# Ignalina/znippy

Hardware: AMD Instinct MI355X
Metric: decompress MB/s (uncompressed) + compress MB/s, 100k x 10KB archive (higher is better)
Workload: dtype u8; 1 GPU; 100k x 10KiB text chunks (BASELINE configs[1]); rows_per_gpu=100000, chunk_bytes=10240, bytes_per_gpu=1024000000, blob_bytes_per_gpu=6400000, parallelism=row-cursor ranges x1, pipelining=step k+1 queued before step k's counters are read (two runs in flight)

## Files before the change

znippy_amd/csrc/api.hip:

```cpp
#include <unistd.h>
#include "common.h"
#include "encode.h"
#include "../../include/znippy_hip.h"

#include <algorithm>
#include <cstdio>
#include <cstdlib>
#include <cstring>
#include <chrono>
#include <memory>
#include <string>
#include <vector>
#include <unordered_map>

namespace zn {
int measure_b3_pass_ns(int cus, hipStream_t s, float *ns_per_pass_per_simd, float *ghz);
size_t decode_lit_scratch_bytes(int grid);
void set_fused_dbg(unsigned long long *p);
void set_fused_abl(int v);
}

using namespace zn;
extern "C" void zn_rounds_totals(const uint64_t *len, const uint8_t *skip, size_t n, uint64_t out[8]);
extern "C" void zn_rows_extents(const uint64_t *bo, const uint64_t *bs, const uint64_t *oo, const uint64_t *us, size_t n, uint64_t out[8]);
// ... 59 lines not shown
    uint16_t *bx_fse_pool = nullptr;
    uint16_t *bx_huf_pool = nullptr;
    uint64_t bx_fse_cap = 0, bx_huf_cap = 0;
    uint32_t *rx_pool = nullptr, *rx_chunk = nullptr;
    uint8_t *rx_cdone = nullptr;
    uint64_t rx_cap = 0;
    uint8_t *vs_pool = nullptr;
    uint64_t vs_cap = 0;
    hipEvent_t ev_fork = nullptr, ev_join = nullptr, ev_join2 = nullptr;
    std::vector<KTime> ktimes;
    int n_ktimes = 0;
    std::vector<hipEvent_t> event_pool;
    bool ktime_open = false;
    std::vector<std::pair<size_t, void *>> pinned_pool;
    size_t pinned_pool_bytes = 0;
    std::vector<std::pair<size_t, void *>> dev_pool;
    std::unordered_map<void *, size_t> dev_sizes;
    size_t dev_pool_bytes = 0;
    struct {
        int dbg = 0;
        unsigned lds_pad = 0;
        int store_g = 0;
        bool no_block_items = false, no_fused_blocks = false, ddbg = false, edbg = false, no_fused_store = false,
             nohash = false, no_roles = false, no_fz = false, fz_only = false, no_bx = false, tdbg = false, no_fuse_hash = false, trace = false, no_rx = false, no_pack = false, no_lean = false, no_stored_only = false;
        unsigned roles_min = 2048;
        unsigned bx_big = BX_BIG_SEQ;
        bool bx_big_set = false;
        int ktime = 2;
    } sw;
    int cus = 256;
    int live_tables = 0;
    bool closing = false;
    unsigned long long *clk_buf = nullptr;
    enum Diag { DIAG_FUSED, DIAG_ITEMS, DIAG_FZ, DIAG_GENERAL, DIAG_BX, DIAG_ENCODE, DIAG_N };
    unsigned long long *diag[DIAG_N] = {};
};

static void read_switches(znippy_ctx *ctx) {
    auto on = [](const char *n) { const char *v = getenv(n); return v && *v && *v != '0'; };
    if (const char *e = getenv("ZNIPPY_DBG")) ctx->sw.dbg = atoi(e);
    if (const char *e = getenv("ZNIPPY_LDS_PAD")) ctx->sw.lds_pad = (unsigned)atoi(e);
    ctx->sw.no_block_items = on("ZNIPPY_NO_BLOCK_ITEMS");
    ctx->sw.no_fused_blocks = on("ZNIPPY_NO_FUSED_BLOCKS");
    ctx->sw.ddbg = on("ZNIPPY_DDBG");
    ctx->sw.edbg = on("ZNIPPY_EDBG");
    ctx->sw.no_fused_store = on("ZNIPPY_NO_FUSED_STORE");
    ctx->sw.nohash = on("ZNIPPY_NOHASH");
    ctx->sw.no_roles = on("ZNIPPY_NO_ROLES");
    ctx->sw.no_fz = on("ZNIPPY_NO_FZ");
    ctx->sw.tdbg = on("ZNIPPY_TDBG");
    ctx->sw.trace = on("ZNIPPY_TRACE");
    ctx->sw.no_lean = on("ZNIPPY_NO_LEAN");
    ctx->sw.no_pack = on("ZNIPPY_NO_PACK");
    if (const char *e = getenv("ZNIPPY_STORE_G")) ctx->sw.store_g = atoi(e) == 1 ? 1 : (atoi(e) == 2 ? 2 : 0);
    ctx->sw.no_stored_only = on("ZNIPPY_NO_STORED_ONLY");
    ctx->sw.no_rx = on("ZNIPPY_NO_RX");
    ctx->sw.no_fuse_hash = on("ZNIPPY_NO_FUSE_HASH");
    ctx->sw.no_bx = on("ZNIPPY_NO_BX");
    if (const char *e = getenv("ZNIPPY_BX_BIG")) { ctx->sw.bx_big = (unsigned)atoi(e); ctx->sw.bx_big_set = true; }
    if (const char *lv = getenv("ZNIPPY_LEVEL")) { const int v = atoi(lv); if (v >= 1 && v <= 22) ctx->level = v; }
    if (const char *wl = getenv("ZNIPPY_WINDOW_LOG")) { const int v = atoi(wl); if (v == 0 || (v >= WINDOW_LOG_MIN && v <= WINDOW_LOG_MAX)) ctx->window_log = v; }
    if (const char *gs = getenv("ZNIPPY_GEN_SHARE")) { const int v = atoi(gs); if (v >= 1 && v <= 4) ctx->gen_share = v; }
    ctx->sw.fz_only = on("ZNIPPY_FZ_ONLY");
    if (const char *e = getenv("ZNIPPY_ROLES_MIN")) ctx->sw.roles_min = (unsigned)atoi(e);
    if (const char *e = getenv("ZNIPPY_KTIME")) ctx->sw.ktime = atoi(e);
}

static void *pinned_take(znippy_ctx *ctx, size_t bytes, size_t *cap) {
    size_t best = ctx->pinned_pool.size();
    for (size_t i = 0; i < ctx->pinned_pool.size(); i++)
        if (ctx->pinned_pool[i].first >= bytes && ctx->pinned_pool[i].first <= 4 * bytes + 4096 &&
            (best == ctx->pinned_pool.size() || ctx->pinned_pool[i].first < ctx->pinned_pool[best].first))
            best = i;
    if (best != ctx->pinned_pool.size()) {
        void *p = ctx->pinned_pool[best].second;
// ... 180 lines not shown
    H_ITEMS = 2,
    H_TILES = 3,
    H_FLAGGED = 5,
};
enum Cursor : uint32_t { CUR_GENERAL = 0, CUR_ROLES = 2, CUR_ITEMS = 4, CUR_FALLBACK = 8, CUR_FZ = 12, CUR_FZ_WORK = 13 };
constexpr uint32_t LEAN_ANY = 1u << H_FUSED | 1u << H_SERIAL | 1u << H_FLAGGED, LEAN_SMALL = LEAN_ANY | 1u << H_TILES, LEAN_BLOCKS = LEAN_ANY | 1u << H_ITEMS;
constexpr bool ctl_before(CtlRegion a, CtlRegion b) { return a.at + a.bytes <= b.at; }
static_assert(ctl_before(CTL_COUNTERS, CTL_HAND) && ctl_before(CTL_HAND, CTL_CURSORS) && ctl_before(CTL_CURSORS, CTL_FZ_POOL) && ctl_before(CTL_FZ_POOL, CTL_BX_POOL) &&
              ctl_before(CTL_BX_POOL, CTL_BX_CTR) && ctl_before(CTL_BX_CTR, CTL_RX) && CTL_RX.at + CTL_RX.bytes <= CTL_HEAD, "control block: regions overlap or pass the head");
static_assert(CTL_COUNTERS.at == 0 && CTL_HAND.at == CTL_COUNTERS.bytes && CTL_MIRROR == CTL_HAND.at + CTL_HAND.bytes, "the mirror is exactly counters + hand-over counts");
static_assert(CTL_FLAG < 8 && H_FLAGGED == H_SERIAL + 4 && H_FLAGGED < 8 && CUR_FZ_WORK < 16 && zn::RX_ROUNDS <= RX_ZERO && RX_ZERO < 16, "control block: a word outside its region");

struct znippy_rows {
    znippy_ctx *ctx = nullptr;
    uint64_t row_begin = 0;
    uint32_t n = 0;
    uint32_t n_compressed = 0;
    uint64_t *blob_off = nullptr, *blob_size = nullptr, *usize = nullptr, *out_off = nullptr;
    uint8_t *compressed = nullptr, *checksum = nullptr, *d_bitmap = nullptr;
    uint32_t *h_pack = nullptr, *d_pack = nullptr;
    size_t h_pack_cap = 0;
    unsigned long long *d_pack_sums = nullptr;
    uint8_t *ctl = nullptr;
    size_t ctl_bytes = 0;
    template <class T> T *ctl_at(CtlRegion g, size_t i = 0) const { return reinterpret_cast<T *>(ctl + g.at) + i; }
    uint32_t *hand(Hand h) const { return ctl_at<uint32_t>(CTL_HAND, h); }
    uint32_t *cur(Cursor c) const { return ctl_at<uint32_t>(CTL_CURSORS, c); }
    int32_t *status = nullptr;
    uint32_t *digests = nullptr;
    uint64_t *counters = nullptr;
    uint64_t *h_counters = nullptr;
    const uint32_t *mirror_hand(unsigned slot) const { return reinterpret_cast<const uint32_t *>(reinterpret_cast<const uint8_t *>(h_counters + 16 * slot) + CTL_HAND.at); }
    size_t h_counters_cap = 0;
    int bx_hint = -1;
    bool lean_ok = false;
    int lean_hint = -1;
    bool lean_blocks_ok = false;
    bool lean_mixed_ok = false;
    bool roles_off = false;
    bool small_ok = false, small_off = false;
    uint32_t *all_rows = nullptr;
    int lean_hint2 = -1;
    struct RunArgs { const void *blobs = nullptr; void *out = nullptr; uint64_t base = 0, cap = 0, blob_cap = ~0ull; bool verify = false; } run_args[2];
    uint64_t *vs_off = nullptr;
    uint64_t vs_bytes = 0;
    bool vs_built = false;
    bool no_out = false;
    hipEvent_t ev_done[2] = {nullptr, nullptr};
    uint64_t run_seq = 0;
    uint64_t ext_min_bo = 0, ext_max_bend = 0, ext_max_oend = 0;
    bool ext_wrap = false;
    std::vector<uint64_t> h_blob_off, h_blob_size, h_len, h_out_off;
    uint64_t blob_cap = ~0ull;
    uint64_t val_base = 0, val_bcap = 0, val_ocap = 0;
    bool val_done = false, val_verify = false;
    uint32_t n_bad = 0;
    bool force_full = false;
    uint8_t *status_init = nullptr;
// ... 805 lines not shown
    r->ctx = ctx;
    ctx->live_tables++;
    r->row_begin = row_begin;
    r->n = (uint32_t)(row_end - row_begin);
    const uint32_t n = r->n;
    bool allc = true;
    if (compressed_bitmap) {
        uint64_t row = row_begin;
        for (; row < row_end && (row & 7); row++) allc &= (compressed_bitmap[row >> 3] >> (row & 7)) & 1;
        for (; row + 8 <= row_end && allc; row += 8) allc &= compressed_bitmap[row >> 3] == 0xFF;
        for (; row < row_end && allc; row++) allc &= (compressed_bitmap[row >> 3] >> (row & 7)) & 1;
    }
    std::vector<uint64_t> own_oo;
    if (!out_offset) {
        r->no_out = true;
        own_oo.resize(n);
        uint64_t at = 0;
        for (uint32_t i = 0; i < n; i++) { own_oo[i] = at; at += uncompressed_size[row_begin + i]; }
    }
    const RowCols c{blob_offset + row_begin, blob_size + row_begin, uncompressed_size + row_begin, out_offset ? out_offset + row_begin : own_oo.data(), compressed_bitmap, row_begin, row_end, allc};
    int rc = rows_columns_h2d(ctx, r, c, checksum, td);
    if (rc) return rc;
    r->corrupt_cap = std::max<uint32_t>(n, 1);
    r->ctl_bytes = CTL_HEAD + std::max<size_t>(4 * (size_t)n, 16);
    if (tmalloc(ctx, &r->ctl, r->ctl_bytes) != hipSuccess ||
        tmalloc(ctx, &r->digests, std::max<size_t>(32 * (size_t)n, 32)) != hipSuccess ||
        !(r->h_counters = (uint64_t *)pinned_take(ctx, 256, &r->h_counters_cap)) ||
        !(r->ev_done[0] = event_take(ctx)) || !(r->ev_done[1] = event_take(ctx)) ||
        tmalloc(ctx, &r->corrupt, 8 * (size_t)r->corrupt_cap) != hipSuccess)
        return ZNIPPY_E_NOMEM;
    r->counters = r->ctl_at<uint64_t>(CTL_COUNTERS);
    r->status = reinterpret_cast<int32_t *>(r->ctl + CTL_HEAD);
    td.mark("allocs");
    PlanBuf p;
    build_plan([=, us = c.us, bs = c.bs, &c](uint32_t i) -> uint64_t { return (allc || c.comp(i)) ? us[i] : bs[i]; }, n, p);
    td.mark("plan");
    if ((rc = upload_plan(ctx, p, r->plan))) return rc;
    td.mark("plan_h2d");
    for (const Tile &t : p.tiles) r->n_small_tiles += t.n_units != 0;
    if (r->n_small_tiles && tmalloc(ctx, &r->slow_list, 4 * (size_t)p.tiles.size()) != hipSuccess) return ZNIPPY_E_NOMEM;
    RowClasses k;
    rows_classify(ctx, r, c, k);
    r->n_list_a = (uint32_t)k.la.size();
    td.mark("big_rows");
    if (r->n_compressed && (rc = rows_batch_buffers(ctx, r, k.nblk))) return rc;
    r->wide_rows = k.n_big && k.big_bytes / k.n_big >= (1u << 20) && k.big_blob * 50 < k.big_bytes;
    r->n_cand = (uint32_t)k.cand_row.size();
    r->n_items = (uint32_t)k.item_row.size();
    const bool hints = !ctx->sw.no_lean && r->n_list_a == 0;
    const uint32_t n_tiles = (uint32_t)p.tiles.size();
    r->small_ok = allc && hints && !ctx->sw.no_bx && r->n_cand == 0 && r->n_small_tiles == n_tiles && r->n_small_tiles > 0 && r->bx_slots;
    r->lean_mixed_ok = hints && r->n_cand == 0 && r->n_small_tiles > 0 && r->n_small_tiles < n_tiles;
    r->lean_blocks_ok = allc && hints && r->n_cand > 0 && r->n_small_tiles == 0;
    r->lean_ok = allc && hints && r->n_cand == 0 && p.big.empty() && r->n_small_tiles == n_tiles && r->n_small_tiles > 0;
    if (r->n_cand && (rc = rows_item_buffers(ctx, r, k))) return rc;
    if (r->n_cand && !ctx->sw.no_fused_blocks && (rc = rows_fused_block_buffers(ctx, r, k, p))) return rc;
    if ((rc = dev_upload(ctx, &r->list_a, k.la.data(), k.la.size()))) return rc;
    if (tmalloc(ctx, &r->pending, std::max<size_t>(4 * (size_t)n, 16)) != hipSuccess) return ZNIPPY_E_NOMEM;
    td.mark("rest");
    *out = guard.release();
    return ZNIPPY_OK;
}
// ... 69 lines not shown
        HIPCHK(ctx, hipMemsetAsync(r->vs_off, 0, 8 * (size_t)r->n, ctx->stream));
    }
    r->vs_built = true;
    return ZNIPPY_OK;
}

static void rows_note_hint(znippy_rows *r, unsigned slot) {
    const uint32_t *left = r->mirror_hand(slot);
    const bool handed = left[H_FUSED] || left[H_SERIAL] || left[H_FLAGGED];
    r->bx_hint = (handed || r->n_list_a) ? 1 : 0;
    r->lean_hint = (handed || left[H_TILES]) ? 0 : 1;
    r->lean_hint2 = (handed || left[H_ITEMS]) ? 0 : 1;
    if (r->n_small_tiles && left[H_TILES] >= r->n_small_tiles) r->roles_off = true;
    if (r->small_ok && left[H_FUSED] >= r->n) r->small_off = true;
    if (r->small_off) r->bx_hint = 1;
}

struct RunPlan {
    bool bx;
    bool small_off;
    bool stored_only;
    bool roles;
    bool lean;
    bool lean_mixed;
    bool decode;
    bool one_stream;
    bool lean_blocks;
    bool behind;
    bool rx;
    bool third;
};
static RunPlan rows_plan(const znippy_ctx *ctx, const znippy_rows *r, int preset) {
    const auto &sw = ctx->sw;
    RunPlan p{};
    p.bx = r->bx_slots && ctx->fz_lit_pool && ctx->fz_seq_pool && ctx->bx_fse_pool && ctx->bx_huf_pool && r->bx_hint != 0;
    p.small_off = p.bx && r->small_off && !r->n_bad && !r->force_full && !sw.dbg;
    p.stored_only = r->n_compressed == 0 && !preset && !sw.dbg && !sw.no_stored_only && !r->force_full;
    const bool may_skip = !preset && !r->force_full;
    if (!p.small_off && !p.stored_only) {
        p.roles = !sw.no_roles && sw.roles_min != 0 && r->n_small_tiles >= sw.roles_min && r->n_small_tiles > 0 && !(sw.dbg & (1 | 2 | 4 | 8 | 128)) && !r->roles_off;
        p.lean_mixed = r->lean_mixed_ok && r->lean_hint == 1 && r->bx_hint == 0 && may_skip && !sw.dbg && !sw.ddbg;
        p.lean = p.roles && r->lean_ok && r->lean_hint == 1 && r->bx_hint == 0 && may_skip && !sw.dbg;
    }
    p.decode = !p.lean && !p.lean_mixed && !p.stored_only;
    if (!p.decode) return p;
    p.one_stream = r->n_cand && r->bx_hint == 0 && r->n_small_tiles == 0;
    p.lean_blocks = p.one_stream && r->lean_blocks_ok && r->lean_hint2 == 1 && may_skip && r->n_bt && !sw.ddbg && !r->fz_total;
    if (!r->n_compressed) return p;
    p.behind = !p.bx && r->n_cand && r->bx_hint == 0;
    p.rx = p.bx && r->rx_base && ctx->rx_pool && r->rx_words;
    p.third = p.bx && r->bx_nblk <= 32768;
    return p;
}

static HashArgs rows_hash_args(const znippy_ctx *ctx, const znippy_rows *r, const RowsRun &run) {
    HashArgs h{};
    h.tiles = r->plan.tiles; h.n_tiles = r->plan.n_tiles;
    h.len = r->usize;
    h.srcA = (const uint8_t *)run.d_blobs; h.offA = r->blob_off; h.baseA = run.blob_base;
    h.srcB = (uint8_t *)run.d_out; h.offB = run.verify ? r->vs_off : r->out_off;
    h.sel = r->compressed; h.status = r->status; h.pending_count = r->hand(H_FUSED);
    h.copy_to_B = run.verify ? 0 : 1;
    h.store_tiles = ctx->sw.store_g;
    h.misaligned_dst = !run.verify && (r->odd_out || ((uintptr_t)run.d_out & 15) != 0);
    h.digests = r->digests; h.tile_cv = r->plan.tile_cv;
// ... 45 lines not shown
    f.h = rows_hash_args(ctx, r, run);
    f.h.pass = 1;
    f.blob_size = r->blob_size; f.out_cap = run.out_cap; f.status = r->status;
    f.preset = run.preset;
    f.pending = r->pending; f.pending_count = r->hand(H_FUSED);
    f.dbg = ctx->sw.dbg;
    if (f.dbg & 8) {
        f.dbg_buf = diag_cycle<8>(ctx, znippy_ctx::DIAG_FUSED, s, nullptr, [](const unsigned long long *h4) {
            if (h4[3]) fprintf(stderr, "[znippy dbg] waves=%llu prologue=%.0f decode=%.0f hash=%.0f | parse+lits=%.0f expand-build=%.0f stream-out=%.0f after-match=%.0f cycles/wave\n", h4[3],
                               (double)h4[0] / h4[3], (double)h4[1] / h4[3], (double)h4[2] / h4[3], (double)h4[6] / h4[3], (double)h4[4] / h4[3], (double)h4[5] / h4[3], (double)h4[7] / h4[3]);
        });
        set_fused_dbg(f.dbg_buf);
    }
    if (f.dbg & 32768) {
        if (!ctx->clk_buf) { (void)hipMalloc(&ctx->clk_buf, 64); (void)hipMemset(ctx->clk_buf, 0, 64); }
        f.dbg_buf = ctx->clk_buf;
    }
    if (f.dbg & (16 | 32 | 64)) set_fused_abl(f.dbg);
    f.lds_pad = ctx->sw.lds_pad;
    const hipStream_t fs = p.lean_mixed ? ctx->aux : s;
    if (p.lean_mixed) {
        HIPCHK(ctx, hipEventRecord(ctx->ev_fork, s));
        HIPCHK(ctx, hipStreamWaitEvent(ctx->aux, ctx->ev_fork, 0));
    }
    if (p.roles) {
        f.cursor = r->cur(CUR_ROLES);
        f.tile_list = r->slow_list;
        f.tile_count = r->hand(H_TILES);
        timed(ctx, run.verify ? "verify_roles" : "decode_verify_roles", fs, [&] { launch_fused_roles(f, ctx->cus, fs, run.verify); });
    }
    if (r->n_small_tiles && !p.lean) timed(ctx, run.verify ? "verify_small" : "decode_verify_fused", fs, [&] { launch_fused_small(f, fs, p.roles ? ctx->cus * 5 : 0, run.verify); });
    if (p.lean_mixed) HIPCHK(ctx, hipEventRecord(ctx->ev_join, ctx->aux));
    return ZNIPPY_OK;
}

static void run_two_phase(znippy_ctx *ctx, znippy_rows *r, const RowsRun &run, hipStream_t ba) {
    FzArgs z{};
    z.cand_row = r->cand_row; z.cand_fzbase = r->fz_base; z.cand_fzcap = r->fz_cap; z.n_cand = r->n_cand;
    z.it_cand = r->fz_it_cand; z.total_items = r->fz_total; z.cand_nb = r->fz_nb; z.items = r->fz_items;
    fill_row_args(z, r, run);
    z.row_flag = r->row_flag;
    z.lit_pool = ctx->fz_lit_pool; z.lit_cap = ctx->fz_lit_cap; z.seq_pool = ctx->fz_seq_pool; z.seq_cap = ctx->fz_seq_cap;
    z.pool_used = r->ctl_at<unsigned long long>(CTL_FZ_POOL);
    z.cursor = r->cur(CUR_FZ);
    if (ctx->sw.ddbg)
        z.dbg = diag_cycle<32>(ctx, znippy_ctx::DIAG_FZ, ctx->stream, ba, [](const unsigned long long *h) {
// ... 170 lines not shown
    if (!r->n_cand) return ZNIPPY_OK;
    if (!p.behind) {
        HIPCHK(ctx, hipStreamWaitEvent(s, ctx->ev_join, 0));
        launch_finish_blocks(rows_scan_args(r, run), s, false);
    }
    decode_rest(ctx, r, a, r->n_cand);
    return ZNIPPY_OK;
}

static void run_second_hash(znippy_ctx *ctx, znippy_rows *r, const RunPlan &p, const RowsRun &run) {
    hipStream_t s = ctx->stream;
    HashArgs h = rows_hash_args(ctx, r, run);
    h.pass = p.stored_only ? 0 : 2;
    h.tile_done = r->n_bt && !p.stored_only ? r->tile_done : nullptr;
    timed(ctx, run.verify ? "blake3_hash_only" : "blake3_second_pass", s, [&] { launch_hash_tiles(h, s); });
    if (r->plan.n_big)
        timed(ctx, "blake3_merge_big", s, [&] {
            launch_merge_big(r->plan.big, r->plan.n_big, r->plan.tile_cv, r->digests, r->plan.grp_big, r->plan.grp_k, r->plan.n_grp, r->plan.max_cvs, s);
        });
}

static int run_verify(znippy_ctx *ctx, znippy_rows *r, const RunPlan &p, const RowsRun &run) {
    hipStream_t s = ctx->stream;
    if (p.lean_mixed) HIPCHK(ctx, hipStreamWaitEvent(s, ctx->ev_join, 0));
    const bool skipped = p.lean || p.lean_blocks || p.lean_mixed;
    timed(ctx, "verify", s, [&] {
        launch_verify(r->digests, r->checksum, r->usize, r->status, r->n, r->row_begin, r->counters, r->corrupt, r->corrupt_cap, s,
                      skipped ? r->ctl_at<uint32_t>(CTL_HAND) : nullptr, (p.lean || p.lean_mixed) ? LEAN_SMALL : LEAN_BLOCKS);
    });
    HIPCHK(ctx, hipMemcpyAsync(r->h_counters + 16 * run.slot, r->counters, CTL_MIRROR, hipMemcpyDeviceToHost, s));
    HIPCHK(ctx, hipEventRecord(r->ev_done[run.slot], s));
    HIPCHK(ctx, hipGetLastError());
    return ZNIPPY_OK;
}

static int rows_launch(znippy_ctx *ctx, znippy_rows *r, const void *d_blobs, uint64_t blob_base, void *d_out, uint64_t out_cap,
                       unsigned slot, bool verify, bool *queued = nullptr) {
    ctx->n_ktimes = 0;
    int rc = ensure_decoder(ctx);
    if (!rc && verify) {
        rc = rows_verify_slots(ctx, r);
        if (!rc) rc = ensure_verify_scratch(ctx, r->vs_bytes);
        d_out = ctx->vs_pool; out_cap = r->vs_bytes;
    }
    if (!rc) rc = rows_validate(ctx, r, blob_base, out_cap, verify);
    if (!rc && r->fz_total) rc = ensure_fz_pools(ctx, r->fz_bytes, r->fz_total);
// ... 665 lines not shown
```

znippy_amd/csrc/common.h:

```cpp
#pragma once
#include <hip/hip_runtime.h>
#include <stdint.h>
#include <stddef.h>

namespace zn {

struct Tile {
    uint32_t first_unit;
    uint32_t n_units;
    uint32_t first_leaf;
    uint32_t n_leaves;
    uint32_t cv_index;
    uint32_t pad;
};

struct BigUnit {
    uint32_t unit;
    uint32_t cv_base;
    uint32_t n_cvs;
    uint32_t pad;
};

struct HashArgs {
    const Tile *tiles;
// ... 26 lines not shown
    const uint32_t *pending_count;
    const uint8_t *blobs;
    uint64_t blob_base;
    const uint64_t *blob_off, *blob_size, *usize, *out_off;
    const uint8_t *compressed;
    uint8_t *out;
    uint64_t out_cap;
    int32_t *status;
    uint32_t n_rows;
    uint32_t *cursor;
    uint8_t *lit_scratch;
    unsigned long long *dbg;
    int block_mode;
    const uint32_t *item_row, *item_k;
    const uint32_t *item_src;
    uint32_t n_items;
    uint32_t *row_flag;
    const uint8_t *item_done;
    const uint32_t *todo, *n_todo;
    uint32_t *seq_scratch;
    int preset;
};

struct FusedArgs {
    HashArgs h;
    const uint64_t *blob_size;
    uint64_t out_cap;
    int32_t *status;
    uint32_t *pending;
    uint32_t *pending_count;
    int dbg;
    unsigned long long *dbg_buf;
    uint32_t lds_pad;
    int preset;
    uint32_t *cursor;
    uint32_t *tile_list;
    uint32_t *tile_count;
};

struct FusedBlocksArgs {
    HashArgs h;
    const uint64_t *blob_size;
    const uint32_t *bt_tile, *bt_item;
    uint32_t n_bt;
    const uint32_t *item_src;
    const uint32_t *row_flag;
    uint8_t *tile_done, *item_done;
    int dbg;
};
void launch_fused_blocks(const FusedBlocksArgs &a, hipStream_t s, bool verify = false);

void launch_hash_tiles(const HashArgs &a, hipStream_t s);
void launch_fused_small(const FusedArgs &a, hipStream_t s, int grid_cap = 0, bool verify = false);
void launch_fused_roles(const FusedArgs &a, int cus, hipStream_t s, bool verify = false);
void init_fused_tables();
void launch_merge_big(const BigUnit *big, uint32_t n_big, uint32_t *tile_cv, uint32_t *digests, const uint32_t *grp_big,
                      const uint32_t *grp_k, uint32_t n_grp, uint32_t max_cvs, hipStream_t s);
void launch_verify(const uint32_t *digests, const uint8_t *checksum, const uint64_t *usize,
                   const int32_t *status, uint32_t n_rows, uint64_t row_begin, uint64_t *counters,
                   uint64_t *corrupt_rows, uint32_t corrupt_cap, hipStream_t s, const uint32_t *lean_lists = nullptr, uint32_t lean_mask = 0);
int decode_grid_size(int device);
void launch_decode(const DecodeArgs &a, int grid, bool wide, hipStream_t s);
struct BlockScanArgs {
    const uint32_t *cand_row, *cand_base, *cand_nblocks;
    uint32_t n_cand;
    const uint8_t *blobs;
    uint64_t blob_base;
    const uint64_t *blob_off, *blob_size, *usize, *out_off;
    uint64_t out_cap;
    uint32_t *item_src;
    uint32_t *row_flag;
    int32_t *status;
    uint32_t *pending, *pending_count;
    int preset;
};
void launch_scan_blocks(const BlockScanArgs &a, hipStream_t s);
void launch_compact_items(const uint8_t *item_done, uint32_t n_items, uint32_t *todo, uint32_t *n_todo, hipStream_t s);
// ... 101 lines not shown
```

znippy_amd/csrc/fused_small.hip:

```cpp
#include "common.h"
#include "hash_dev.h"

#include <algorithm>
#include <cstring>

namespace zn {

constexpr uint32_t EOFF_MAX = 960;
constexpr uint32_t EBUF = EOFF_MAX + 1024 + 64;
constexpr int F_E_CORRUPT = -5, F_E_UNSUP = -6, F_E_DST = -4;
constexpr int F_NOT_SIMPLE = 1;

struct DTab {
    uint16_t next;
    uint8_t nbits, addbits;
    uint32_t base;
};
__constant__ DTab c_dll[64], c_dml[64], c_dof[32];
__constant__ uint32_t c_llb[36] = {0, 1, 2, 3, 4, 5, 6, 7, 8, 9, 10, 11, 12, 13, 14, 15, 16, 18,
                                   20, 22, 24, 28, 32, 40, 48, 64, 128, 256, 512, 1024, 2048,
                                   4096, 8192, 16384, 32768, 65536};
__constant__ uint8_t c_lla[36] = {0, 0, 0, 0, 0, 0, 0, 0, 0, 0, 0, 0, 0, 0, 0, 0, 1, 1,
                                  1, 1, 2, 2, 3, 3, 4, 6, 7, 8, 9, 10, 11, 12, 13, 14, 15, 16};
__constant__ uint32_t c_mlb[53] = {3, 4, 5, 6, 7, 8, 9, 10, 11, 12, 13, 14, 15, 16, 17, 18, 19, 20,
// ... 967 lines not shown
                else fq.fold_and_write(s_nodes, a.h);
            }
        }
        if (base + gridDim.x * 4 < n_work) lds_barrier();
    }
    if (clk) { a.dbg_buf[0] = __builtin_amdgcn_s_memtime() - c0; a.dbg_buf[1] = __builtin_amdgcn_s_memrealtime() - r0; }
}

#ifndef ZN_R_SLOTS
#define ZN_R_SLOTS 32
#endif
#ifndef ZN_R_WAVES
#define ZN_R_WAVES 16
#endif
#ifndef ZN_R_LOADERS
#define ZN_R_LOADERS 1
#endif
#ifndef ZN_R_LOADER_EMITS
#define ZN_R_LOADER_EMITS 0
#endif
constexpr uint32_t R_SLOTS = ZN_R_SLOTS, R_GROUP = 4, R_WAVES = ZN_R_WAVES, R_LOADERS = ZN_R_LOADERS;
constexpr bool R_LOADER_EMITS = ZN_R_LOADER_EMITS != 0;
static_assert((R_SLOTS & (R_SLOTS - 1)) == 0 && R_SLOTS >= 2 * R_GROUP, "ring size: a power of two, at least two groups");
constexpr uint32_t R_SLOT_BYTES = WROWS * WSTRIDE;
constexpr uint32_t R_SLOT_NODES = R_SLOT_BYTES / 32;
static_assert(R_SLOT_BYTES % 32 == 0 && R_SLOT_BYTES >= 64 * 32, "a slot must hold 64 chaining values, node-aligned");

typedef __attribute__((address_space(3))) uint32_t lds_u32;
__device__ __forceinline__ uint32_t lds_ld(const uint32_t *p) { return __builtin_amdgcn_readfirstlane(*(const volatile lds_u32 *)p); }
__device__ __forceinline__ void lds_st(uint32_t *p, uint32_t v) { *(volatile lds_u32 *)p = v; }
__device__ __forceinline__ void lds_fence() { asm volatile("s_waitcnt lgkmcnt(0)" ::: "memory"); }

struct alignas(16) RolesShared {
    uint8_t slots[R_SLOTS][R_SLOT_BYTES];
    __attribute__((aligned(16))) uint32_t tree[R_WAVES - R_LOADERS][64 * 8];
    uint64_t oo[R_SLOTS][WROWS];
    uint32_t len[R_SLOTS][WROWS];
    uint32_t tn[R_SLOTS][WROWS], toff[R_SLOTS][WROWS];
    uint16_t dy[R_SLOTS][WROWS], dB[R_SLOTS][WROWS], doff[R_SLOTS][WROWS];
    uint32_t first[R_SLOTS], nunits[R_SLOTS], nleaves[R_SLOTS];
    uint32_t ready, take, finished;
    uint32_t next_iter;
    uint32_t cnt[R_SLOTS / R_GROUP];
    uint32_t gen[R_SLOTS / R_GROUP];
};

__device__ __forceinline__ void emit_periodic_row(uint8_t *Y, uint32_t L0, uint32_t off, float inv, uint8_t *out, uint32_t osize,
                                                  uint32_t lane) {
    const uint32_t B = L0 - off, lim = L0 + 64;
    Y[L0 + lane] = Y[B + lmod(lane, off, inv)];
    const uint32_t head = (uint32_t)((16 - ((uintptr_t)out & 15)) & 15);
    const uint32_t body16 = (osize - head) >> 4;
    const uint32_t step = smod(1024, off), rb = smod(B, off);
    if (lane < head) out[lane] = Y[lane];
    const uint32_t tail = (osize - head) & 15, p = head + 16 * body16 + lane;
    if (lane < tail) {
        uint32_t rt = lmod(p, off, inv) + off - rb;
        if (rt >= off) rt -= off;
        out[p] = p < lim ? Y[p] : Y[B + rt];
    }
    uint32_t x = head + 16 * lane;
    uint32_t r = lmod(x, off, inv) + off - rb;
    if (r >= off) r -= off;
    for (uint32_t i0 = 0; i0 < body16; i0 += 256) {
        const uint32_t i = i0 + lane;
        uint4 v0 = make_uint4(0, 0, 0, 0), v1 = v0, v2 = v0, v3 = v0;
        const uint32_t r0 = r;
// ... 16 lines not shown
}

template <bool STORE>
__device__ __forceinline__ void roles_loader(const FusedArgs &a, RolesShared &S) {
    const uint32_t lane = threadIdx.x & 63, j = lane >> 4, u = lane & 15;
    FastTabs T;
    {
        const DTab eL = c_dll[lane], eM = c_dml[lane], eO = c_dof[lane & 31];
        T.ll = eL.base | (uint32_t)eL.addbits << 24;
        T.ml = eM.base | (uint32_t)eM.addbits << 24;
        T.of = eO.addbits;
        T.lls = lane < 36 ? c_llb[lane] | (uint32_t)c_lla[lane] << 24 : 0u;
        T.mls = lane < 53 ? c_mlb[lane] | (uint32_t)c_mla[lane] << 24 : 0u;
    }
    for (;;) {
        const uint32_t iter = uni(atomicAdd(&S.next_iter, lane == 0 ? 1u : 0u));
        const uint32_t base = uni(atomicAdd(a.cursor, lane == 0 ? R_GROUP : 0u));
        const bool last = base >= a.h.n_tiles;
        const uint32_t grp = iter & (R_SLOTS / R_GROUP - 1), use = iter / (R_SLOTS / R_GROUP);
        const uint32_t ti = base + j;
        Tile t{0, 0, 0, 0, 0, 0};
        if (ti < a.h.n_tiles) t = a.h.tiles[ti];
        const bool small = t.n_units >= 1;
        const bool cand = small && t.n_units <= WROWS;
        const bool rowv = cand && u < t.n_units;
        uint32_t c_sel = 0, c_bs = 0;
        uint64_t c_len = 0, c_src = 0, c_oo = 0;
        int32_t c_st = 0;
        if (rowv) {
            const uint32_t row = t.first_unit + u;
            if (a.preset) c_st = a.status[row];
            c_sel = a.h.sel[row];
            c_len = a.h.len[row];
            c_src = a.h.offA[row] - a.h.baseA;
            if (STORE) c_oo = a.h.offB[row];
            const uint64_t bs = a.blob_size[row];
            c_bs = bs > 0xFFFFFFFFull ? 0xFFFFFFFFu : (uint32_t)bs;
        }
        const bool want = rowv && c_sel && c_st == 0 && c_len != 0 && (c_len & 1023) == 0 && c_len <= 0x10000 &&
                          (!STORE || c_oo + c_len <= a.out_cap) && c_bs >= 12 && c_bs <= WIN;
        while (lds_ld(&S.gen[grp]) != use) __builtin_amdgcn_s_sleep(4);
        asm volatile("" ::: "memory");
        const uint32_t slot = grp * R_GROUP + j;
        uint8_t *const win = S.slots[slot] + (u < WROWS ? u : 0) * WSTRIDE;
        const uint8_t *const src = a.h.srcA + c_src;
        const uint32_t nb = want ? c_bs : 0, full = nb >> 4, tail = nb & 15;
// ... 251 lines not shown
            FoldQueue<4> fq;
            fq.n_tab = 64;
            fq.tb_n = uu < WROWS ? S.tn[sl][uu] : 0u;
            fq.tb_off = uu < WROWS ? S.toff[sl][uu] : 0u;
            fq.tb_out = S.first[sl] + uu;
            fq.tb_root = 1;
            if (__ballot(fq.tb_n != 0) != 0ull && !(a.dbg & 131072)) {
                uint32_t *const nodes = reinterpret_cast<uint32_t *>(S.slots[grp * R_GROUP]);
                FoldQueue<4> fd = fq.dense16();
                uint32_t U = 0;
                const uint32_t n = (a.dbg & 262144) ? 0u : fd.uniform(&U);
                if (n) fd.fold_uniform_and_write(nodes, h, n, U);
                else fq.fold_and_write(nodes, h);
            }
            lds_fence();
            if (lane == 0) {
                lds_st(&S.cnt[grp], 0u);
                lds_st(&S.gen[grp], lds_ld(&S.gen[grp]) + 1u);
            }
        }
    }
}

template <bool STORE>
__global__ __launch_bounds__(R_WAVES * 64) void k_fused_roles(FusedArgs a) {
    extern __shared__ __attribute__((aligned(16))) uint8_t s_roles_raw[];
    RolesShared &S = *reinterpret_cast<RolesShared *>(s_roles_raw);
    if (threadIdx.x == 0) { S.ready = 0; S.take = 0; S.finished = 0; S.next_iter = 0; }
    if (threadIdx.x < R_SLOTS / R_GROUP) { S.cnt[threadIdx.x] = 0; S.gen[threadIdx.x] = 0; }
    __syncthreads();
    const bool clk = (a.dbg & 32768) && a.dbg_buf && blockIdx.x == 7 && threadIdx.x == 64 * R_LOADERS;
    const unsigned long long c0 = clk ? __builtin_amdgcn_s_memtime() : 0, r0 = clk ? __builtin_amdgcn_s_memrealtime() : 0;
    if (threadIdx.x < 64 * R_LOADERS) {
        if (!(a.dbg & 64)) __builtin_amdgcn_s_setprio(3);
        roles_loader<STORE>(a, S);
    } else roles_hasher<STORE>(a, S);
    if (clk) { a.dbg_buf[0] = __builtin_amdgcn_s_memtime() - c0; a.dbg_buf[1] = __builtin_amdgcn_s_memrealtime() - r0; }
}

void launch_fused_roles(const FusedArgs &a, int cus, hipStream_t s, bool verify) {
    if (!a.h.n_tiles) return;
    static bool attr_set[2] = {false, false};
    if (!attr_set[verify]) {
        (void)hipFuncSetAttribute(verify ? reinterpret_cast<const void *>(k_fused_roles<false>) : reinterpret_cast<const void *>(k_fused_roles<true>),
                                  hipFuncAttributeMaxDynamicSharedMemorySize, (int)sizeof(RolesShared));
        attr_set[verify] = true;
    }
    const uint32_t want = (a.h.n_tiles + R_GROUP - 1) / R_GROUP;
    const uint32_t per_cu = sizeof(RolesShared) > 80 * 1024 ? 1u : 2u;
    uint32_t grid = std::min<uint32_t>((uint32_t)cus * per_cu, want);
    if (a.lds_pad) grid = std::min<uint32_t>(grid, a.lds_pad);
    if (verify) hipLaunchKernelGGL(k_fused_roles<false>, dim3(grid), dim3(R_WAVES * 64), sizeof(RolesShared), s, a);
    else hipLaunchKernelGGL(k_fused_roles<true>, dim3(grid), dim3(R_WAVES * 64), sizeof(RolesShared), s, a);
}

template <bool STORE>
__global__ __launch_bounds__(256, 4) void k_fused_blocks(FusedBlocksArgs a) {
    __shared__ __attribute__((aligned(16))) uint8_t s_area[4][STAGE_FULL_BYTES];
    uint32_t *const s_nodes = reinterpret_cast<uint32_t *>(&s_area[0][0]);
    constexpr uint32_t AREA_NODES = STAGE_FULL_BYTES / 32;
    static_assert(STAGE_FULL_BYTES % 32 == 0, "area must be a whole number of nodes");
    __shared__ uint32_t s_tab[3][4 * FOLD_UNITS];
    __shared__ __attribute__((aligned(16))) uint8_t s_Wb[4][WSTRIDE];
    __shared__ uint16_t s_d[4][3];
    const uint32_t lane = threadIdx.x & 63, w = threadIdx.x >> 6;
    if (lane < FOLD_UNITS) s_tab[0][w * FOLD_UNITS + lane] = 0;
    const uint32_t idx = blockIdx.x * 4 + w;
    if (idx < a.n_bt) {
        const uint32_t ti = a.bt_tile[idx], item = a.bt_item[idx];
        const Tile t = a.h.tiles[ti];
        const uint32_t row = t.first_unit;
        const uint32_t src_pos = a.item_src[item];
        const uint64_t usize = a.h.len[row];
        const uint64_t origin = (uint64_t)(t.first_leaf >> 7) << 17;
// ... 92 lines not shown
```

Measured before the change: 1.961 million MB/s.

## Fuse checksum verification and counter tally into the tail of the roles kernel

Each roles workgroup now records which tiles it processed in LDS. After hashing, it compares the row digests against the expected checksums, tallies lengths, ok, corrupt and failed counts, and reduces them into sharded global counters. The last workgroup to arrive, found with a ticket atomic, writes the final counters and the hand-over mirror, so the separate verify launch is skipped. This removes a kernel launch and a second pass over the digests. In exchange it adds LDS per block, a tail phase after the main work and a grid-wide atomic ticket, and it only applies when the record buffer fits.

```diff
diff --git a/znippy_amd/csrc/api.hip b/znippy_amd/csrc/api.hip
--- a/znippy_amd/csrc/api.hip
+++ b/znippy_amd/csrc/api.hip
@@ -105,7 +105,7 @@
         unsigned lds_pad = 0;
         int store_g = 0;
         bool no_block_items = false, no_fused_blocks = false, ddbg = false, edbg = false, no_fused_store = false,
-             nohash = false, no_roles = false, no_fz = false, fz_only = false, no_bx = false, tdbg = false, no_fuse_hash = false, trace = false, no_rx = false, no_pack = false, no_lean = false, no_stored_only = false;
+             nohash = false, no_roles = false, no_fz = false, fz_only = false, no_bx = false, tdbg = false, no_fuse_hash = false, trace = false, no_rx = false, no_pack = false, no_lean = false, no_tail = false, no_stored_only = false;
         unsigned roles_min = 2048;
         unsigned bx_big = BX_BIG_SEQ;
         bool bx_big_set = false;
@@ -134,6 +134,7 @@
     ctx->sw.tdbg = on("ZNIPPY_TDBG");
     ctx->sw.trace = on("ZNIPPY_TRACE");
     ctx->sw.no_lean = on("ZNIPPY_NO_LEAN");
+    ctx->sw.no_tail = on("ZNIPPY_NO_TAIL");
     ctx->sw.no_pack = on("ZNIPPY_NO_PACK");
     if (const char *e = getenv("ZNIPPY_STORE_G")) ctx->sw.store_g = atoi(e) == 1 ? 1 : (atoi(e) == 2 ? 2 : 0);
     ctx->sw.no_stored_only = on("ZNIPPY_NO_STORED_ONLY");
@@ -360,7 +361,7 @@
     size_t h_pack_cap = 0;
     unsigned long long *d_pack_sums = nullptr;
     uint8_t *ctl = nullptr;
-    size_t ctl_bytes = 0;
+    size_t ctl_bytes = 0, tail_at = 0;
     template <class T> T *ctl_at(CtlRegion g, size_t i = 0) const { return reinterpret_cast<T *>(ctl + g.at) + i; }
     uint32_t *hand(Hand h) const { return ctl_at<uint32_t>(CTL_HAND, h); }
     uint32_t *cur(Cursor c) const { return ctl_at<uint32_t>(CTL_CURSORS, c); }
@@ -372,6 +373,7 @@
     size_t h_counters_cap = 0;
     int bx_hint = -1;
     bool lean_ok = false;
+    uint64_t tile_rows = 0;
     int lean_hint = -1;
     bool lean_blocks_ok = false;
     bool lean_mixed_ok = false;
@@ -1223,7 +1225,8 @@
     int rc = rows_columns_h2d(ctx, r, c, checksum, td);
     if (rc) return rc;
     r->corrupt_cap = std::max<uint32_t>(n, 1);
-    r->ctl_bytes = CTL_HEAD + std::max<size_t>(4 * (size_t)n, 16);
+    r->tail_at = (CTL_HEAD + std::max<size_t>(4 * (size_t)n, 16) + 127) & ~(size_t)127;
+    r->ctl_bytes = r->tail_at + zn::TAIL_BYTES;
     if (tmalloc(ctx, &r->ctl, r->ctl_bytes) != hipSuccess ||
         tmalloc(ctx, &r->digests, std::max<size_t>(32 * (size_t)n, 32)) != hipSuccess ||
         !(r->h_counters = (uint64_t *)pinned_take(ctx, 256, &r->h_counters_cap)) ||
@@ -1238,7 +1241,7 @@
     td.mark("plan");
     if ((rc = upload_plan(ctx, p, r->plan))) return rc;
     td.mark("plan_h2d");
-    for (const Tile &t : p.tiles) r->n_small_tiles += t.n_units != 0;
+    for (const Tile &t : p.tiles) { r->n_small_tiles += t.n_units != 0; r->tile_rows += t.n_units; }
     if (r->n_small_tiles && tmalloc(ctx, &r->slow_list, 4 * (size_t)p.tiles.size()) != hipSuccess) return ZNIPPY_E_NOMEM;
     RowClasses k;
     rows_classify(ctx, r, c, k);
@@ -1354,6 +1357,7 @@
     bool stored_only;
     bool roles;
     bool lean;
+    bool tail;
     bool lean_mixed;
     bool decode;
     bool one_stream;
@@ -1373,6 +1377,7 @@
         p.roles = !sw.no_roles && sw.roles_min != 0 && r->n_small_tiles >= sw.roles_min && r->n_small_tiles > 0 && !(sw.dbg & (1 | 2 | 4 | 8 | 128)) && !r->roles_off;
         p.lean_mixed = r->lean_mixed_ok && r->lean_hint == 1 && r->bx_hint == 0 && may_skip && !sw.dbg && !sw.ddbg;
         p.lean = p.roles && r->lean_ok && r->lean_hint == 1 && r->bx_hint == 0 && may_skip && !sw.dbg;
+        p.tail = p.lean && !sw.no_tail && r->checksum && r->tile_rows == r->n && fused_roles_tail_fits(r->plan.n_tiles, ctx->cus, sw.lds_pad);
     }
     p.decode = !p.lean && !p.lean_mixed && !p.stored_only;
     if (!p.decode) return p;
@@ -1464,6 +1469,18 @@
     if (p.lean_mixed) {
         HIPCHK(ctx, hipEventRecord(ctx->ev_fork, s));
         HIPCHK(ctx, hipStreamWaitEvent(ctx->aux, ctx->ev_fork, 0));
+    }
+    if (p.tail) {
+        zn::RolesTail &t = f.tail;
+        t.shards = reinterpret_cast<unsigned long long *>(r->ctl + r->tail_at);
+        t.counters = reinterpret_cast<unsigned long long *>(r->counters);
+        t.hand = r->ctl_at<uint32_t>(CTL_HAND);
+        t.lean_mask = LEAN_SMALL;
+        t.corrupt_cap = r->corrupt_cap;
+        t.checksum = r->checksum;
+        t.corrupt = r->corrupt;
+        t.row_begin = r->row_begin;
+        t.mirror = reinterpret_cast<unsigned long long *>(r->h_counters + 16 * run.slot);
     }
     if (p.roles) {
         f.cursor = r->cur(CUR_ROLES);
@@ -1680,6 +1697,11 @@
 
 static int run_verify(znippy_ctx *ctx, znippy_rows *r, const RunPlan &p, const RowsRun &run) {
     hipStream_t s = ctx->stream;
+    if (p.tail) {
+        HIPCHK(ctx, hipEventRecord(r->ev_done[run.slot], s));
+        HIPCHK(ctx, hipGetLastError());
+        return ZNIPPY_OK;
+    }
     if (p.lean_mixed) HIPCHK(ctx, hipStreamWaitEvent(s, ctx->ev_join, 0));
     const bool skipped = p.lean || p.lean_blocks || p.lean_mixed;
     timed(ctx, "verify", s, [&] {
diff --git a/znippy_amd/csrc/common.h b/znippy_amd/csrc/common.h
--- a/znippy_amd/csrc/common.h
+++ b/znippy_amd/csrc/common.h
@@ -72,8 +72,23 @@
     int preset;
 };
 
+constexpr uint32_t TAIL_SHARDS = 16;
+constexpr size_t TAIL_BYTES = (TAIL_SHARDS + 1) * 128;
+struct RolesTail {
+    unsigned long long *shards;
+    unsigned long long *counters;
+    uint32_t *hand;
+    uint32_t lean_mask;
+    uint32_t corrupt_cap;
+    const uint8_t *checksum;
+    uint64_t *corrupt;
+    uint64_t row_begin;
+    unsigned long long *mirror;
+};
+
 struct FusedArgs {
     HashArgs h;
+    RolesTail tail;
     const uint64_t *blob_size;
     uint64_t out_cap;
     int32_t *status;
@@ -103,6 +118,7 @@
 void launch_hash_tiles(const HashArgs &a, hipStream_t s);
 void launch_fused_small(const FusedArgs &a, hipStream_t s, int grid_cap = 0, bool verify = false);
 void launch_fused_roles(const FusedArgs &a, int cus, hipStream_t s, bool verify = false);
+bool fused_roles_tail_fits(uint32_t n_tiles, int cus, uint32_t grid_cap);
 void init_fused_tables();
 void launch_merge_big(const BigUnit *big, uint32_t n_big, uint32_t *tile_cv, uint32_t *digests, const uint32_t *grp_big,
                       const uint32_t *grp_k, uint32_t n_grp, uint32_t max_cvs, hipStream_t s);
diff --git a/znippy_amd/csrc/fused_small.hip b/znippy_amd/csrc/fused_small.hip
--- a/znippy_amd/csrc/fused_small.hip
+++ b/znippy_amd/csrc/fused_small.hip
@@ -1013,6 +1013,7 @@
 constexpr uint32_t R_SLOTS = ZN_R_SLOTS, R_GROUP = 4, R_WAVES = ZN_R_WAVES, R_LOADERS = ZN_R_LOADERS;
 constexpr bool R_LOADER_EMITS = ZN_R_LOADER_EMITS != 0;
 static_assert((R_SLOTS & (R_SLOTS - 1)) == 0 && R_SLOTS >= 2 * R_GROUP, "ring size: a power of two, at least two groups");
+constexpr uint32_t R_REC = 128;
 constexpr uint32_t R_SLOT_BYTES = WROWS * WSTRIDE;
 constexpr uint32_t R_SLOT_NODES = R_SLOT_BYTES / 32;
 static_assert(R_SLOT_BYTES % 32 == 0 && R_SLOT_BYTES >= 64 * 32, "a slot must hold 64 chaining values, node-aligned");
@@ -1034,6 +1035,8 @@
     uint32_t next_iter;
     uint32_t cnt[R_SLOTS / R_GROUP];
     uint32_t gen[R_SLOTS / R_GROUP];
+    uint32_t rec_first[R_REC][R_GROUP], rec_rows[R_REC][R_GROUP];
+    uint32_t rec_over;
 };
 
 __device__ __forceinline__ void emit_periodic_row(uint8_t *Y, uint32_t L0, uint32_t off, float inv, uint8_t *out, uint32_t osize,
@@ -1096,6 +1099,10 @@
         Tile t{0, 0, 0, 0, 0, 0};
         if (ti < a.h.n_tiles) t = a.h.tiles[ti];
         const bool small = t.n_units >= 1;
+        if (u == 0) {
+            if (iter < R_REC) { S.rec_first[iter][j] = t.first_unit; S.rec_rows[iter][j] = t.n_units; }
+            else if (!last) S.rec_over = 1u;
+        }
         const bool cand = small && t.n_units <= WROWS;
         const bool rowv = cand && u < t.n_units;
         uint32_t c_sel = 0, c_bs = 0;
@@ -1393,11 +1400,104 @@
     }
 }
 
+
+struct RolesTailArgs {
+    const uint64_t *len;
+    const uint32_t *digests;
+    const int32_t *status;
+};
+#define ZN_GLOBAL __attribute__((address_space(1)))
+template <class T> __device__ __forceinline__ ZN_GLOBAL T *as_global(T *p) { return (ZN_GLOBAL T *)p; }
+template <class T> __device__ __forceinline__ T dev_add(ZN_GLOBAL T *p, T v) { return __hip_atomic_fetch_add(p, v, __ATOMIC_RELAXED, __HIP_MEMORY_SCOPE_AGENT); }
+template <class T> __device__ __forceinline__ T dev_load(ZN_GLOBAL T *p) { return __hip_atomic_load(p, __ATOMIC_RELAXED, __HIP_MEMORY_SCOPE_AGENT); }
+__device__ __forceinline__ void roles_tail(const RolesTailArgs &h, const RolesTail &t, RolesShared &S) {
+#if defined(__HIP_DEVICE_COMPILE__)
+    ZN_GLOBAL const uint64_t *const g_len = as_global(h.len);
+    ZN_GLOBAL const int32_t *const g_status = as_global(h.status);
+    ZN_GLOBAL const uint4 *const g_want = as_global(reinterpret_cast<const uint4 *>(t.checksum));
+    ZN_GLOBAL const uint4 *const g_got = as_global(reinterpret_cast<const uint4 *>(h.digests));
+    ZN_GLOBAL unsigned long long *const g_shards = as_global(t.shards), *const g_counters = as_global(t.counters), *const g_mirror = as_global(t.mirror);
+    ZN_GLOBAL uint32_t *const g_hand = as_global(t.hand);
+    ZN_GLOBAL uint64_t *const g_corrupt = as_global(t.corrupt);
+    __builtin_amdgcn_fence(__ATOMIC_RELEASE, "workgroup");
+    __syncthreads();
+    __builtin_amdgcn_fence(__ATOMIC_ACQUIRE, "workgroup");
+    const uint32_t lane = threadIdx.x & 63, w = threadIdx.x >> 6;
+    const uint32_t iters = lds_ld(&S.next_iter), n_rec = iters < R_REC ? iters : R_REC;
+    unsigned long long v[6] = {0, 0, 0, 0, 0, 0};
+    const uint32_t u = threadIdx.x & 15;
+    for (uint32_t k = threadIdx.x >> 4; k < n_rec * R_GROUP; k += R_WAVES * 4) {
+        const uint32_t first = S.rec_first[k / R_GROUP][k % R_GROUP], rows = S.rec_rows[k / R_GROUP][k % R_GROUP];
+        for (uint32_t q = u; q < rows; q += 16) {
+            const uint32_t r = first + q;
+            ZN_GLOBAL const uint4 *want = g_want + (size_t)r * 2, *got = g_got + (size_t)r * 2;
+            const int32_t st = g_status[r];
+            const unsigned long long len = g_len[r];
+            const uint4 w0 = want[0], w1 = want[1], g0 = got[0], g1 = got[1];
+            v[0] += 1;
+            if (st < 0) {
+                v[5] += 1;
+                continue;
+            }
+            v[1] += len;
+            const bool ok = w0.x == g0.x && w0.y == g0.y && w0.z == g0.z && w0.w == g0.w &&
+                            w1.x == g1.x && w1.y == g1.y && w1.z == g1.z && w1.w == g1.w;
+            if (ok) v[2] += len;
+            else {
+                v[3] += len;
+                v[4] += 1;
+                const unsigned long long slot = dev_add(&g_counters[6], 1ull);
+                if (t.corrupt && slot < t.corrupt_cap) g_corrupt[slot] = t.row_begin + r;
+            }
+        }
+    }
+    unsigned long long *const red = reinterpret_cast<unsigned long long *>(&S.slots[0][0]);
+#pragma unroll
+    for (int c = 0; c < 6; c++) {
+        unsigned long long x = v[c];
+#pragma unroll
+        for (int d = 32; d >= 1; d >>= 1) x += __shfl_xor(x, d);
+        if (lane == 0) red[c * R_WAVES + w] = x;
+    }
+    __syncthreads();
+    if (w != 0) return;
+    unsigned long long x = 0;
+    if (lane < 6)
+        for (uint32_t i = 0; i < R_WAVES; i++) x += red[lane * R_WAVES + i];
+    if (lane == 7) x = S.rec_over;
+    unsigned long long old = 0;
+    if (lane < 8 && x) old = dev_add(&g_shards[(blockIdx.x % TAIL_SHARDS) * 16 + lane], x);
+    asm volatile("s_waitcnt vmcnt(0)" : "+v"(old) : : "memory");
+    ZN_GLOBAL uint32_t *const ticket = as_global(reinterpret_cast<uint32_t *>(t.shards + TAIL_SHARDS * 16));
+    const uint32_t arrived = uni(dev_add(ticket, lane == 0 ? 1u : 0u));
+    if (arrived != gridDim.x - 1) return;
+    static_assert(TAIL_SHARDS == 16, "two reads of eight shards each");
+    const unsigned long long s0 = dev_load(&g_shards[(lane >> 3) * 16 + (lane & 7)]);
+    const unsigned long long s1 = dev_load(&g_shards[(8 + (lane >> 3)) * 16 + (lane & 7)]);
+    const uint32_t hv = dev_load(&g_hand[lane & 15]);
+    const unsigned long long listed = dev_load(&g_counters[6]);
+    unsigned long long tot = s0 + s1;
+#pragma unroll
+    for (int d = 8; d <= 32; d <<= 1) tot += __shfl_xor(tot, d);
+    const bool over = __shfl(tot, 7) != 0;
+    const bool left = __ballot(lane < 8 && ((t.lean_mask >> lane) & 1u) && hv != 0u) != 0ull;
+    const unsigned long long c = lane < 6 ? tot : (lane == 6 ? listed : ((over || left) ? 1ull : 0ull));
+    const uint32_t h_lo = __shfl(hv, (2 * lane) & 15), h_hi = __shfl(hv, (2 * lane + 1) & 15);
+    if (lane < 8) {
+        g_counters[lane] = c;
+        g_mirror[lane] = c;
+    } else if (lane < 16) {
+        g_mirror[lane] = (unsigned long long)h_hi << 32 | h_lo;
+    }
+#endif
+}
+#undef ZN_GLOBAL
+
 template <bool STORE>
 __global__ __launch_bounds__(R_WAVES * 64) void k_fused_roles(FusedArgs a) {
     extern __shared__ __attribute__((aligned(16))) uint8_t s_roles_raw[];
     RolesShared &S = *reinterpret_cast<RolesShared *>(s_roles_raw);
-    if (threadIdx.x == 0) { S.ready = 0; S.take = 0; S.finished = 0; S.next_iter = 0; }
+    if (threadIdx.x == 0) { S.ready = 0; S.take = 0; S.finished = 0; S.next_iter = 0; S.rec_over = 0; }
     if (threadIdx.x < R_SLOTS / R_GROUP) { S.cnt[threadIdx.x] = 0; S.gen[threadIdx.x] = 0; }
     __syncthreads();
     const bool clk = (a.dbg & 32768) && a.dbg_buf && blockIdx.x == 7 && threadIdx.x == 64 * R_LOADERS;
@@ -1407,6 +1507,38 @@
         roles_loader<STORE>(a, S);
     } else roles_hasher<STORE>(a, S);
     if (clk) { a.dbg_buf[0] = __builtin_amdgcn_s_memtime() - c0; a.dbg_buf[1] = __builtin_amdgcn_s_memrealtime() - r0; }
+#if defined(__HIP_DEVICE_COMPILE__)
+    typedef __attribute__((address_space(4))) const unsigned long long karg_u64;
+    karg_u64 *kp = (karg_u64 *)__builtin_amdgcn_kernarg_segment_ptr();
+    asm volatile("" : "+s"(kp));
+    auto word = [&](size_t off) { return kp[off / 8]; };
+    struct Words { unsigned long long w[sizeof(RolesTail) / 8]; } tw;
+    static_assert(sizeof(RolesTail) == sizeof(Words) && offsetof(FusedArgs, tail) % 8 == 0, "the tail's block: whole 64-bit words");
+#pragma unroll
+    for (size_t i = 0; i < sizeof(RolesTail) / 8; i++) tw.w[i] = word(offsetof(FusedArgs, tail) + 8 * i);
+    const RolesTail t = __builtin_bit_cast(RolesTail, tw);
+    if (!t.shards) return;
+    static_assert(offsetof(FusedArgs, h.len) % 8 == 0 && offsetof(FusedArgs, h.digests) % 8 == 0 && offsetof(FusedArgs, status) % 8 == 0, "read as 64-bit words");
+    const RolesTailArgs h{reinterpret_cast<const uint64_t *>(word(offsetof(FusedArgs, h.len))),
+                          reinterpret_cast<const uint32_t *>(word(offsetof(FusedArgs, h.digests))),
+                          reinterpret_cast<const int32_t *>(word(offsetof(FusedArgs, status)))};
+    roles_tail(h, t, S);
+#endif
+}
+
+static uint32_t fused_roles_grid(uint32_t n_tiles, int cus, uint32_t grid_cap) {
+    const uint32_t want = (n_tiles + R_GROUP - 1) / R_GROUP;
+    const uint32_t per_cu = sizeof(RolesShared) > 80 * 1024 ? 1u : 2u;
+    uint32_t grid = std::min<uint32_t>((uint32_t)cus * per_cu, want);
+    if (grid_cap) grid = std::min<uint32_t>(grid, grid_cap);
+    return grid;
+}
+
+bool fused_roles_tail_fits(uint32_t n_tiles, int cus, uint32_t grid_cap) {
+    const uint32_t grid = fused_roles_grid(n_tiles, cus, grid_cap);
+    if (!grid) return false;
+    const uint32_t groups = (n_tiles + R_GROUP - 1) / R_GROUP;
+    return 2 * ((groups + grid - 1) / grid) + 8 <= R_REC;
 }
 
 void launch_fused_roles(const FusedArgs &a, int cus, hipStream_t s, bool verify) {
@@ -1417,10 +1549,7 @@
                                   hipFuncAttributeMaxDynamicSharedMemorySize, (int)sizeof(RolesShared));
         attr_set[verify] = true;
     }
-    const uint32_t want = (a.h.n_tiles + R_GROUP - 1) / R_GROUP;
-    const uint32_t per_cu = sizeof(RolesShared) > 80 * 1024 ? 1u : 2u;
-    uint32_t grid = std::min<uint32_t>((uint32_t)cus * per_cu, want);
-    if (a.lds_pad) grid = std::min<uint32_t>(grid, a.lds_pad);
+    const uint32_t grid = fused_roles_grid(a.h.n_tiles, cus, a.lds_pad);
     if (verify) hipLaunchKernelGGL(k_fused_roles<false>, dim3(grid), dim3(R_WAVES * 64), sizeof(RolesShared), s, a);
     else hipLaunchKernelGGL(k_fused_roles<true>, dim3(grid), dim3(R_WAVES * 64), sizeof(RolesShared), s, a);
 }
```

After: 1.965 million MB/s, median of 4. No clear change (+0.2%).
